# HKUST-Aerial-Robotics/VINS-Mobile

Measured on AMD Instinct MI355X. Metric: VIO frames/sec (KLT+window solve), 640x480/150 feats/W=10, higher is better.
Workload: dtype f64 (solve) / u8+i32+f32 (KLT)

## Files before the change

### vins-mobile_amd/abi.py

```python
import ctypes as C
import os

import numpy as np

VIO_OK = 0
VIO_EINVAL, VIO_ENODEV, VIO_ENOMEM, VIO_ECAP, VIO_ESTATE, VIO_ETIMEOUT = -1, -2, -3, -4, -5, -6
VIO_MAX_PRIOR_BLOCKS = 96
VIO_MAX_TRACE = 64
VIO_INIT_BA_MAX_FRAMES = 32
VIO_BLOCK_POSE, VIO_BLOCK_SPEEDBIAS, VIO_BLOCK_EXPOSE = 0, 1, 2
VIO_MARGIN_OLD, VIO_MARGIN_SECOND_NEW, VIO_MARGIN_NONE = 0, 1, 2
STAGES = ["setup_imu", "setup_prior", "eval_prior", "eval_imu", "eval_proj", "scale", "schur", "rhs", "cholesky",
          "tri_solve", "quad_form", "dogleg", "cost_eval", "new2old", "marg_build", "marg_chol", "total",
          "p_zero", "p_fact", "p_gram", "p_feat", "c_potrf", "c_trsm", "imu_raw", "c_wait", "q_w", "backsolve",
          "c_ahead", "tr_vec", "m_prior", "m_imu", "m_fact", "m_gram", "d0", "d1", "d2", "d3", "d4", "d5",
          "v_gd", "v_dot", "v_step", "v_plus", "v_gmax", "v_rest", "b_init", "b_pose", "b_asp", "b_band", "b_gn",
          "e_head", "e_copy", "e_h0dx", "e_tail", "x0", "x1", "x2", "x3"]

_dp = C.POINTER(C.c_double)
_ip = C.POINTER(C.c_int32)


class VioConfig(C.Structure):
    _fields_ = [
        ("window_size", C.c_int32), ("max_features", C.c_int32), ("max_factors", C.c_int32),
        ("max_iterations", C.c_int32), ("image_rows", C.c_int32), ("image_cols", C.c_int32),
        ("max_corners", C.c_int32), ("min_dist", C.c_int32), ("freq", C.c_int32),
        ("lk_win", C.c_int32), ("lk_levels", C.c_int32), ("lk_max_iters", C.c_int32),
        ("lk_eps", C.c_double), ("lk_min_eig", C.c_double), ("quality_level", C.c_double),
        ("f_threshold", C.c_double), ("f_confidence", C.c_double),
        ("fx", C.c_double), ("fy", C.c_double), ("cx", C.c_double), ("cy", C.c_double),
        ("gravity", C.c_double), ("acc_n", C.c_double), ("acc_w", C.c_double),
        ("gyr_n", C.c_double), ("gyr_w", C.c_double), ("cauchy_a", C.c_double),
    ]


def hip_runtime(lib=None):
    lib = lib or load_product()
    buf, n = C.create_string_buffer(4096), C.c_int32()
    lib.vio_hip_runtime(buf, 4096, C.byref(n))
    return [p for p in buf.value.decode().split(";") if p]


def host_pool_width():
    lib = load_product()
    n = C.c_int32(0)
    return int(lib.vio_host_pool_width(C.byref(n))), int(n.value)


def default_config(**kw):
    c = VioConfig(
        window_size=10, max_features=1000, max_factors=8192, max_iterations=10,
        image_rows=640, image_cols=480, max_corners=70, min_dist=30, freq=3,
        lk_win=21, lk_levels=3, lk_max_iters=30, lk_eps=0.01, lk_min_eig=1e-4,
        quality_level=0.01, f_threshold=1.0, f_confidence=0.99,
        fx=526.600, fy=526.678, cx=243.481, cy=315.280,
        gravity=9.805, acc_n=0.5, acc_w=0.002, gyr_n=0.2, gyr_w=4.0e-5, cauchy_a=1.0)
    for k, v in kw.items():
        setattr(c, k, v)
    return c


class VioPreintegration(C.Structure):
    _fields_ = [
        ("sum_dt", C.c_double), ("delta_p", C.c_double * 3), ("delta_q", C.c_double * 4),
        ("delta_v", C.c_double * 3), ("linearized_ba", C.c_double * 3),
        ("linearized_bg", C.c_double * 3), ("jacobian", C.c_double * 225),
        ("covariance", C.c_double * 225),
    ]


PREINT_DOUBLES = C.sizeof(VioPreintegration) // 8


class VioPrior(C.Structure):
    _fields_ = [
        ("n", C.c_int32), ("n_blocks", C.c_int32),
        ("block_kind", C.c_int32 * VIO_MAX_PRIOR_BLOCKS),
        ("block_index", C.c_int32 * VIO_MAX_PRIOR_BLOCKS),
        ("block_offset", C.c_int32 * VIO_MAX_PRIOR_BLOCKS),
        ("block_x0", _dp), ("linearized_jacobians", _dp), ("linearized_residuals", _dp),
    ]


class VioWindow(C.Structure):
    _fields_ = [
        ("window_size", C.c_int32), ("n_features", C.c_int32), ("n_factors", C.c_int32),
        ("marginalization_flag", C.c_int32),
        ("pose", _dp), ("speed_bias", _dp), ("ex_pose", _dp), ("inv_depth", _dp),
        ("factor_host", _ip), ("factor_target", _ip), ("factor_feature", _ip),
        ("factor_pts_i", _dp), ("factor_pts_j", _dp),
        ("preint", C.POINTER(VioPreintegration)), ("prior", C.POINTER(VioPrior)),
        ("loop_frame", C.c_int32), ("loop_pose", _dp),
        ("use_origin_override", C.c_int32), ("origin_yaw_deg", C.c_double),
        ("origin_p", C.c_double * 3),
        ("raw_pose", _dp), ("raw_speed_bias", _dp), ("raw_inv_depth", _dp),
        ("next_prior", C.POINTER(VioPrior)),
        ("resident_prior", C.c_int32),
    ]

# ... 481 lines not shown
```

### vins-mobile_amd/csrc/solver_core.h

```cpp
#pragma once

#include <math.h>
#include <stdint.h>

#include <type_traits>

#include "solve_trace.h"
#include "vio_math.h"

#include "spmd.h"
#include "factors.h"
#include "mfma_tiles.h"

namespace vio {

constexpr int kBS = 15;
constexpr int kSS = kSB * kSB;
constexpr int kAW = 18;
constexpr int kAS = kSB * kAW;

struct WinView {
  int W, P, F, M, np, nblk, has_loop, loop_frame, marg_flag, max_iter;
  int prior_n, prior_nb;
  int Fpad;
// ... 200 lines not shown
  const int need = (n + 4 * kStrip - 1) / (4 * kStrip);
  nparts = nparts < need ? need : (nparts > 8 ? 8 : nparts);
  const int per = (n + nparts - 1) / nparts;
  VIO_PARFOR(q, n * nparts) {
    const int part = q / n, c = q - part * n;
    const int k0 = part * per, k1 = k0 + per < n ? k0 + per : n;
    double xs[kStrip], s = 0;
    for (int b0 = k0; b0 < k1; b0 += kStrip) {
      const int nb = k1 - b0 < kStrip ? k1 - b0 : kStrip;
#pragma unroll
      for (int j = 0; j < kStrip; j++) xs[j] = M[(size_t)(b0 + (j < nb ? j : 0)) * n + c];
      VIO_SCHED_FENCE();
#pragma unroll
      for (int j = 0; j < kStrip; j++) s += (j < nb ? xs[j] : 0.0) * x[b0 + (j < nb ? j : 0)];
    }
    if (k1 > k0) add(c, s);
  }
}


template <class MP>
VIO_DEV void setup_imu_info_gj(const Ctx &cx, const WinView &v, MP mbox) {
  const int W = v.W;
  const int tid_ = VIO_TID(cx), j = tid_ & 31, slot = tid_ >> 5, nslots = cx.nt >> 5;
  for (int f0 = 0; f0 < W; f0 += nslots) {
    const int f = f0 + slot;
    const bool act = f < W && j < 30;
    const int fc = f < W ? f : 0;
    auto mb = mbox + slot * 32;
    double x[15];
#pragma unroll
    for (int r = 0; r < 15; r++)
      x[r] = j < 15 ? v.preint[fc * kPreintDoubles + 242 + r * 15 + (j < 15 ? j : 0)] : (double)(j - 15 == r);
#pragma unroll
    for (int c = 0; c < 15; c++) {
      if (j == c) {
        int piv = c;
        double best = fabs(x[c]);
#pragma unroll
        for (int r = c + 1; r < 15; r++)
          if (fabs(x[r]) > best) best = fabs(x[r]), piv = r;
#pragma unroll
        for (int r = 0; r < 15; r++) mb[r] = x[r];
        mb[15] = (double)piv;
      }
      __builtin_amdgcn_fence(__ATOMIC_RELEASE, "wavefront");
      __builtin_amdgcn_wave_barrier();
      __builtin_amdgcn_fence(__ATOMIC_ACQUIRE, "wavefront");
      const int piv = (int)mb[15];
      double m[15];
#pragma unroll
      for (int r = 0; r < 15; r++) m[r] = mb[r];
      __builtin_amdgcn_wave_barrier();
      double xp = x[c], mp = m[c];
#pragma unroll
      for (int r = 0; r < 15; r++) {
        if (r == piv) xp = x[r], mp = m[r];
      }
#pragma unroll
      for (int r = 0; r < 15; r++) {
        if (r == piv && r != c) x[r] = x[c], m[r] = m[c];
      }
      const double d = mp;
      x[c] = xp / d;
#pragma unroll
      for (int r = 0; r < 15; r++) {
        if (r != c) {
          const double fac = m[r];
          if (fac != 0.0) x[r] -= fac * x[c];
        }
      }
    }
    if (act && j >= 15) {
      const int cc = j - 15;
#pragma unroll
      for (int rr = 0; rr < 15; rr++)
        if (rr >= cc) v.imu_info[f * 225 + rr * 15 + cc] = x[rr], v.imu_info[f * 225 + cc * 15 + rr] = x[rr];
    }
  }
  VIO_SYNC();
}

template <class WK>
VIO_DEV void setup_prior(const Ctx &cx, const WinView &v, WK &w) {
  const int n = v.prior_n;
  if (n <= 0) return;
  VIO_PARFOR(a, n) w.prcol[a] = -1;
  VIO_SYNC();
  VIO_PARFOR(b, v.prior_nb) {
    int kind = v.pr_kind[b], idx = v.pr_index[b], o = v.pr_offset[b];
    if (kind == 0)
      for (int k = 0; k < 6; k++) w.prcol[o + k] = (idx << 8) | k;
    else if (kind == 1)
      for (int k = 0; k < 9; k++) w.prcol[o + k] = (idx << 8) | (6 + k);
  }
  const bool stage = (size_t)n * n <= (size_t)w.nstage;
  auto Js = w.stage;
  if (stage) {
    VIO_PARFOR(q, n * n) Js[q] = v.pr_J[q];
    VIO_SYNC();
  }
  {
    const int tid_ = VIO_TID(cx), wave = __builtin_amdgcn_readfirstlane(tid_ >> 6), nw = cx.nt >> 6, lane = tid_ & 63;
    const int li = lane & 15, kq = lane >> 4;
    const int nt16 = (n + 15) >> 4, ntiles = nt16 * (nt16 + 1) / 2, ksteps = (n + 3) >> 2;
    for (int t = wave; t < ntiles; t += nw) {
      int ti = 0;
      while ((ti + 1) * (ti + 2) / 2 <= t) ti++;
      const int tj = t - ti * (ti + 1) / 2;
      const int ca = 16 * ti + li, cb = 16 * tj + li;
      const bool va = ca < n, vb = cb < n;
      const int oa = va ? ca : 0, ob = vb ? cb : 0;
      v4d acc0 = {0.0, 0.0, 0.0, 0.0}, acc1 = {0.0, 0.0, 0.0, 0.0};
      constexpr int kChunk = 8;
      for (int s0 = 0; s0 < ksteps; s0 += kChunk) {
        double av[kChunk], bv[kChunk];
#pragma unroll
        for (int j = 0; j < kChunk; j++) {
          const int k = 4 * (s0 + j) + kq, kc = k < n ? k : 0;
          if (stage) av[j] = Js[kc * n + oa], bv[j] = Js[kc * n + ob];
          else av[j] = v.pr_J[kc * n + oa], bv[j] = v.pr_J[kc * n + ob];
        }
        __builtin_amdgcn_sched_barrier(0);
#pragma unroll
        for (int j = 0; j < kChunk; j++) {
          const bool vk = 4 * (s0 + j) + kq < n;
          av[j] = (va && vk) ? av[j] : 0.0, bv[j] = (vb && vk) ? bv[j] : 0.0;
        }
#pragma unroll
        for (int j = 0; j < kChunk; j += 2) acc0 = mfma_f64(av[j], bv[j], acc0), acc1 = mfma_f64(av[j + 1], bv[j + 1], acc1);
      }
      acc0 += acc1;
#pragma unroll
      for (int r = 0; r < 4; r++) {
        const int a = 16 * ti + kq + 4 * r, b = cb;
        if (a < n && b < n) {
          v.prH0[a * n + b] = acc0[r];
          if (ti != tj) v.prH0[b * n + a] = acc0[r];
        }
      }
    }
  }
  VIO_PARFOR(a, n) {
    double s = 0;
    if (stage) {
      for (int k = 0; k < n; k++) s = fma(Js[k * n + a], v.pr_r[k], s);
    } else {
      for (int k = 0; k < n; k++) s = fma(v.pr_J[k * n + a], v.pr_r[k], s);
    }
    v.prb0[a] = s;
  }
  const int napp = (int)tri_doubles(v.nrows), nband = 2 * v.P * kSS;
  VIO_PARFOR(q, kSB * v.jp) v.Apri[q] = 0.0;
  VIO_PARFOR(q, napp + nband) v.AppPr[q] = 0.0;
  VIO_SYNC();
  VIO_PARFOR(q, n * n) {
    const int a = q / n, b = q - a * n, pa = w.prcol[a], pb = w.prcol[b];
    if (pa < 0 || pb < 0 || pa < pb) continue;
    const int fr = pa >> 8, cr = pa & 255, fc = pb >> 8, cc = pb & 255;
    const double x = v.prH0[q];
    if (cr < 6 && cc < 6) v.AppPr[tri_at(6 * fr + cr, 6 * fc + cc)] = x;
    else if (cr >= 6 && cc >= 6) {
      if (fr == fc) v.AppPr[napp + fr * kSS + (cr - 6) * kSB + (cc - 6)] = x;
      else if (fr - fc == 1) v.AppPr[napp + v.P * kSS + fr * kSS + (cc - 6) * kSB + (cr - 6)] = x;
    } else if (cr >= 6) v.Apri[(cr - 6) * v.jp + 6 * fc + cc] = x;
    else v.Apri[(cc - 6) * v.jp + 6 * fr + cr] = x;
  }
  VIO_SYNC();
}

template <class MP>
VIO_DEV void setup_imu_info(const Ctx &cx, const WinView &v, MP mbox) {
  const int W = v.W;
  VIO_PARFOR(q, W * 450) v.imu_J[q] = 0.0;
  constexpr int kLd = 17, kTile = 16 * kLd + 16;
  const int tid_ = VIO_TID(cx), wave = __builtin_amdgcn_readfirstlane(tid_ >> 6), nw = cx.nt >> 6, lane = tid_ & 63;
  const int n = lane & 15, kq = lane >> 4;
  auto T = mbox + wave * kTile;
  auto ldv = T + 16 * kLd;
  bool all_good = true;
  if (cx.tid == 0) mbox[nw * kTile] = 0.0;
  VIO_SYNC();
  for (int f = wave; f < W; f += nw) {
    const double *cov = v.preint + f * kPreintDoubles + 242;
    double c4[4];
#pragma unroll
    for (int r = 0; r < 4; r++) {
      const int row = kq + 4 * r, hi = row > n ? row : n, lo = row > n ? n : row;
      c4[r] = cov[(hi < 15 ? hi : 0) * 15 + (lo < 15 ? lo : 0)];
    }
#pragma unroll
    for (int r = 0; r < 4; r++) {
      const int row = kq + 4 * r;
      T[row * kLd + n] = (row < 15 && n < 15) ? c4[r] : (row == n ? 1.0 : 0.0);
    }
    __builtin_amdgcn_fence(__ATOMIC_RELEASE, "wavefront");
    __builtin_amdgcn_wave_barrier();
    __builtin_amdgcn_fence(__ATOMIC_ACQUIRE, "wavefront");
    const bool good = potrf16_wave(T, T, kLd, 15, 15, false, ldv, lane);
    all_good = all_good && good;
    __builtin_amdgcn_fence(__ATOMIC_RELEASE, "wavefront");
    __builtin_amdgcn_wave_barrier();
    __builtin_amdgcn_fence(__ATOMIC_ACQUIRE, "wavefront");
    double x[4];
    const double dg = ldv[n < 15 ? n : 0];
#pragma unroll
    for (int s4 = 0; s4 < 4; s4++) x[s4] = T[(n < 15 ? n : 0) * kLd + (4 * s4 + kq)];
    VIO_SCHED_FENCE();
    v4d acc = {0.0, 0.0, 0.0, 0.0};
#pragma unroll
    for (int s4 = 0; s4 < 4; s4++) {
      const int k = 4 * s4 + kq;
      const double xv = (n < 15 && k < 15) ? (k > n ? x[s4] : (k == n ? dg : 0.0)) : 0.0;
      acc = mfma_f64(xv, xv, acc);
    }
#pragma unroll
    for (int r = 0; r < 4; r++) {
      const int row = kq + 4 * r;
      if (row < 15 && n < 15) v.imu_info[f * 225 + row * 15 + n] = acc[r];
    }
    __builtin_amdgcn_wave_barrier();
  }
  if (__builtin_amdgcn_ballot_w64(!all_good) != 0 && lane == 0) mbox[nw * kTile] = 1.0;
  VIO_SYNC();
  const bool fallback = mbox[nw * kTile] == 1.0;
  VIO_SYNC();
  if (fallback) setup_imu_info_gj(cx, v, mbox);
}

constexpr int kPanelTiles = 5;
constexpr int kGRow = 10;
constexpr int kGSlot = 2 * kGRow + 1;
constexpr int kGramPiece = 30;
constexpr int kGramMinChunk = 32;

template <class WK>
VIO_DEV int gram_chunk_slots(const Ctx &cx, const WK &w) {
  int CH = (w.nstage / kGSlot) & ~1;
  if (CH >= (int)cx.nt) CH -= CH % (int)cx.nt;
  return CH;
}

template <class WK>
VIO_DEV void build_gram_pieces(const Ctx &cx, const WinView &v, WK &w) {
  const int CH = gram_chunk_slots(cx, w), nchunks = (v.nslots + CH - 1) / CH;
  ldsi cnt = reinterpret_cast<ldsi>(w.stage);
  ldsi cc = cnt + v.npairs;
  VIO_PARFOR(c, nchunks + 1) cc[c] = 0;
  VIO_SYNC();
  VIO_PARFOR(b, v.npairs) {
    const int s0 = v.pair_s0[b], s1 = v.pair_s1[b];
    int n = 0;
    for (int c = s0 / CH; c * CH < s1; c++) {
      const int lo = s0 > c * CH ? s0 : c * CH, hi = s1 < (c + 1) * CH ? s1 : (c + 1) * CH;
      const int np_ = (hi - lo + kGramPiece - 1) / kGramPiece;
      n += np_;
#ifdef VIO_HOST_BUILD
      cc[c + 1] += np_;
#else
      __hip_atomic_fetch_add(cc + c + 1, np_, __ATOMIC_RELAXED, __HIP_MEMORY_SCOPE_WORKGROUP);
#endif
    }
    cnt[b] = n;
  }
  VIO_SYNC();
// ... 1984 lines not shown
      relin = true;
      continue;
    }
    invalid_run = 0;
    stamp(cx, ST_DOGLEG);
    const bool speculate = last_ok;
    const int npose7 = (v.P + v.has_loop) * 7, o_sb = 7 * (v.P + 1), o_f = o_sb + 9 * v.P, o_v = o_f + F, nv = v.nblk * kBS;
    double step_norm, cand_norm;
    {
      double d2 = 0, c2 = 0, dummy3 = 0;
      plus_in_place(cx, fresh(), w, w.t2, w.tf, v.stash, o_sb, o_f, d2, c2);
      VIO_PARFOR(q, F)
        v.stash[o_v + 3 * nv + q] = w.gf[q], v.stash[o_v + 3 * nv + F + q] = w.hff[q], v.stash[o_v + 3 * nv + 2 * F + q] = w.gnf[q];
      VIO_PARFOR(i, np) v.stash[o_v + i] = w.gp[i], v.stash[o_v + nv + i] = w.dp[i], v.stash[o_v + 2 * nv + i] = w.gnp[i];
      block_sum3(cx, d2, c2, dummy3);
      step_norm = sqrt(d2), cand_norm = sqrt(c2);
      stamp(cx, ST_V_PLUS);
    }
    double cand_cost = evaluate(cx, fresh(), w, w.xpose, w.xsb, w.xfeat, speculate, true, false, !speculate);
    if (!isfinite(cand_cost)) cand_cost = 1.7976931348623157e308;
    auto restore_iterate = [&]() {
      VIO_PARFOR(q, npose7) w.xpose[q] = v.stash[q];
      VIO_PARFOR(q, v.P * 9) w.xsb[q] = v.stash[o_sb + q];
      VIO_PARFOR(q, F) w.xfeat[q] = v.stash[o_f + q];
    };
    if (step_norm <= 1e-8 * (x_norm + 1e-8)) {
      restore_iterate();
      termination = 1;
      break;
    }
    double cost_change = x_cost - cand_cost;
    if (fabs(cost_change) <= 1e-6 * x_cost) {
      restore_iterate();
      termination = 1;
      break;
    }
    const double rho = step_quality(ev, cand_cost, model_cost_change);
    if (rho > 1e-3) {
      x_norm = cand_norm;
      x_cost = cand_cost;
      if (rho < 0.25) radius *= 0.5;
      if (rho > 0.75) radius = fmax(radius, 3.0 * dogleg_step_norm);
      mu = fmax(min_mu, 2.0 * mu / mu_inc);
      reuse = false;
      ev.current_cost = cand_cost, ev.accumulated_candidate_model_cost_change += model_cost_change, ev.accumulated_reference_model_cost_change += model_cost_change;
      if (ev.current_cost < ev.minimum_cost) ev.minimum_cost = ev.current_cost, ev.candidate_cost = ev.current_cost, ev.accumulated_candidate_model_cost_change = 0;
      else if (ev.current_cost > ev.candidate_cost) ev.candidate_cost = ev.current_cost, ev.accumulated_candidate_model_cost_change = 0;
      ev.reference_cost = ev.candidate_cost, ev.accumulated_reference_model_cost_change = ev.accumulated_candidate_model_cost_change;
      last_ok = true;
      n_ok++;
      recorded = it + 1, min_rec = fmin(min_rec, x_cost);
      if (speculate) {
        gmax = grad_max_norm();
        if (cx.tid == 0) trace.record(it, x_cost, radius, step_norm, rho, gmax, true, true);
        stamp(cx, ST_V_GMAX);
      } else {
        relin = true, relin_reuse = true, rec_pending = true;
        rec_it = it, rec_step_norm = step_norm, rec_rho = rho;
      }
    } else {
      radius *= 0.5;
      reuse = true;
      last_ok = false;
      n_bad++;
      if (cx.tid == 0) trace.record(it, cand_cost, radius, step_norm, rho, 0.0, true, false);
      recorded = it + 1, min_rec = fmin(min_rec, cand_cost);
      restore_iterate();
      if (speculate) {
        VIO_PARFOR(q, F) w.gf[q] = v.stash[o_v + 3 * nv + q], w.hff[q] = v.stash[o_v + 3 * nv + F + q], w.gnf[q] = v.stash[o_v + 3 * nv + 2 * F + q];
        VIO_PARFOR(i, np) w.gp[i] = v.stash[o_v + i], w.dp[i] = v.stash[o_v + nv + i], w.gnp[i] = v.stash[o_v + 2 * nv + i];
      }
      VIO_SYNC();
      stamp(cx, ST_V_REST);
    }
  }
  if (cx.tid == 0) trace.finish(recorded, termination, n_ok, n_bad, min_rec);
  VIO_SYNC();
}

template <class WK>
VIO_DEV void init_band_reach(const Ctx &cx, const WinView &v, WK &w) {
  VIO_PARFOR(k, v.P) {
    int lo = 6 * (k > 0 ? k - 1 : 0), pr = 0;
    for (int b = 0; b < v.prior_nb; b++)
      if (v.pr_kind[b] == 1 && v.pr_index[b] == k) lo = 0, pr = 1;
    w.sbr[2 * k] = lo, w.sbr[2 * k + 1] = pr;
  }
}

#ifndef VIO_HOST_BUILD
template <class WK>
VIO_DEV void coop_helper(const Ctx &cx, const WinView &v, WK &w) {
  const CoopLayout L = CoopLayout::make(v.Pcap, v.Fcap, v.nblk_cap);
  const int np = v.np, F = v.F, nFr = v.P + v.has_loop;
  const size_t fs = ((size_t)v.Fcap + 7) & ~(size_t)7;
  double *part = v.coop + L.o_part + (size_t)(cx.member - 1) * L.part;
  init_band_reach(cx, v, w);
  VIO_SYNC();
  for (;;) {
    const int cmd = coop_wait_cmd(cx, v);
    if (cmd == COOP_EVAL) {
      VIO_PARFOR(q, 7 * nFr) w.xpose[q] = v.coop[L.o_pose + q];
      VIO_PARFOR(q, F) w.xfeat[q] = v.coop[L.o_feat + q];
      VIO_PARFOR(q, 7) w.ex[q] = v.coop[L.o_ex + q];
      VIO_PARFOR(q, np) w.gp[q] = 0.0;
      VIO_PARFOR(q, F) {
        w.gf[q] = 0.0, w.hff[q] = 0.0;
        w.cfeat[q] = w.stf[q] = w.gnf[q] = w.tf[q] = w.ef[q] = w.einv[q] = 0.0;
      }
      VIO_PARFOR(q, nFr * 36) w.ppd[q] = 0.0;
      VIO_SYNC();
      VIO_PARFOR(i, nFr + 1) {
        const bool is_ex = i == nFr;
        double R[9];
        if (is_ex) qtoR(Quat{w.ex[3], w.ex[4], w.ex[5], w.ex[6]}, R);
        else qtoR(Quat{w.xpose[7 * i + 3], w.xpose[7 * i + 4], w.xpose[7 * i + 5], w.xpose[7 * i + 6]}, R);
        auto dst = w.rot + 9 * (is_ex ? v.P + 1 : i);
        for (int k = 0; k < 9; k++) dst[k] = R[k];
      }
      VIO_SYNC();
      const double cost = block_sum(cx, projections_jac(cx, v, w, w.xpose, w.xfeat, true, cx.member, cx.coop, false));
      ldsd whv[6] = {w.cfeat, w.stf, w.gnf, w.tf, w.ef, w.einv};
      VIO_PARFOR(q, np) part[L.p_gp + q] = w.gp[q];
      VIO_PARFOR(q, nFr * 36) part[L.p_ppd + q] = w.ppd[q];
      VIO_PARFOR(f, F) {
        part[L.p_f + f] = w.hff[f], part[L.p_f + fs + f] = w.gf[f];
#pragma unroll
        for (int c = 0; c < 6; c++) part[L.p_f + (2 + c) * fs + f] = whv[c][f];
      }
      if (cx.tid == 0) part[L.p_cost] = cost;
    } else if (cmd == COOP_SCHUR) {
      VIO_PARFOR(f, F) w.einv[f] = v.coop[L.o_einv + f], w.tf[f] = v.coop[L.o_tf + f];
      VIO_SYNC();
      schur_general(cx, v, w, cx.member, cx.coop);
    } else if (cmd == COOP_SYRK) {
      band_syrk_share(cx, v, w, cx.member, cx.coop);
    } else {
      break;
    }
    coop_done(cx, v);
  }
}
#endif

template <bool REGS, int NW, class WK, class VP, class WP>
VIO_DEV void solve_window(const Ctx &cx, const WinView &v, WK &w, const VP &fresh, const WP &fresh_work) {
  const int P = v.P, F = v.F;
  VIO_PARFOR(q, P * 7) w.xpose[q] = v.pose0[q];
  VIO_PARFOR(q, P * 9) w.xsb[q] = v.sb0[q];
  VIO_PARFOR(q, F) w.xfeat[q] = v.feat0[q];
  VIO_PARFOR(q, 7) w.ex[q] = v.ex[q];
  if (v.has_loop) VIO_PARFOR(q, 7) w.xpose[7 * P + q] = v.pose0[7 * v.loop_frame + q];
  VIO_PARFOR(q, v.nblk * kBS) w.t1[q] = 0.0, w.t2[q] = 0.0;
  if (cx.tid == 0) w.flag[0] = w.flag[1] = w.flag[2] = w.flag[3] = 0;
  init_band_reach(cx, v, w);
  VIO_SYNC();
  if (cx.prof && cx.tid == cx.prof_tid) {
    for (int q = 0; q < ST_COUNT; q++) cx.lprof[q] = 0;
    cx.lprof[ST_COUNT - 1] = clock64();
    cx.lprof[ST_TOTAL] = -cx.lprof[ST_COUNT - 1];
  }
  VIO_PARFOR(q, v.nslots) v.sfact[q] = -1;
  VIO_SYNC();
  VIO_PARFOR(q, v.nslots) v.srec_i[q] = -1;
  VIO_SYNC();
  VIO_PARFOR(k, v.M) {
    const int sl = v.fslot[k];
    v.sfact[sl] = k;
    v.srec_i[sl] = v.fhost[k] | (v.ftarget[k] << 8) | (v.ffeat[k] << 16);
    double *d = v.srec_d + 6 * (size_t)sl;
    for (int c = 0; c < 3; c++) d[c] = v.pts_i[3 * k + c], d[3 + c] = v.pts_j[3 * k + c];
  }
  build_gram_pieces(cx, v, w);
  VIO_PARFOR(f, F) w.fh[f] = v.fstart[f + 1] > v.fstart[f] ? v.fhost[v.fstart[f]] : -1;
  VIO_PARFOR(q, (int)tri_doubles(v.nrows)) v.PP[q] = 0.0;
  setup_imu_info(cx, fresh(), w.stage);
  stamp(cx, ST_SETUP_IMU);
  setup_prior(cx, fresh(), w);
  stamp(cx, ST_SETUP_PRIOR);

  minimize<REGS, NW>(cx, v, w, fresh, fresh_work);

  VIO_PARFOR(q, P * 7) v.raw_pose[q] = w.xpose[q];
  VIO_PARFOR(q, P * 9) v.raw_sb[q] = w.xsb[q];
  VIO_PARFOR(q, F) v.raw_feat[q] = w.xfeat[q];
  if (v.has_loop) VIO_PARFOR(q, 7) v.out_loop[q] = w.xpose[7 * P + q];
  VIO_SYNC();
  double R0in[9], ypr0[3], R00[9], ypr00[3], rot_diff[9];
  qtoR(qnormalized(qfrom_pose(v.pose0)), R0in);
  R2ypr(R0in, ypr0);
  double origin_yaw = v.use_origin ? v.origin_yaw : ypr0[0];
  double op[3] = {v.use_origin ? v.origin_p[0] : v.pose0[0], v.use_origin ? v.origin_p[1] : v.pose0[1],
                  v.use_origin ? v.origin_p[2] : v.pose0[2]};
  qtoR(qfrom_pose(w.xpose), R00);
  R2ypr(R00, ypr00);
  double yd[3] = {origin_yaw - ypr00[0], 0, 0};
  ypr2R(yd, rot_diff);
  double p0[3] = {w.xpose[0], w.xpose[1], w.xpose[2]};
  VIO_SYNC();
  VIO_PARFOR(i, P) {
    auto pp = w.xpose + 7 * i, sbv = w.xsb + 9 * i;
    double Rq[9], Rs[9], d[3] = {pp[0] - p0[0], pp[1] - p0[1], pp[2] - p0[2]}, Ps[3], Vs[3];
    qtoR(qnormalized(qfrom_pose(pp)), Rq);
    mat3mul(rot_diff, Rq, Rs);
    mat3vec(rot_diff, d, Ps);
    double vv[3] = {sbv[0], sbv[1], sbv[2]};
    mat3vec(rot_diff, vv, Vs);
    Quat q = RtoQ(Rs);
    auto po = w.cpose + 7 * i, so = w.csb + 9 * i;
    for (int k = 0; k < 3; k++) po[k] = Ps[k] + op[k], so[k] = Vs[k];
    po[3] = q.x, po[4] = q.y, po[5] = q.z, po[6] = q.w;
    for (int k = 3; k < 9; k++) so[k] = sbv[k];
  }
  VIO_PARFOR(f, F) {
    double estimated_depth = 1.0 / w.xfeat[f];
    w.cfeat[f] = 1. / estimated_depth;
  }
  VIO_SYNC();
  VIO_PARFOR(q, P * 7) v.out_pose[q] = w.cpose[q], w.xpose[q] = w.cpose[q];
  VIO_PARFOR(q, P * 9) v.out_sb[q] = w.csb[q], w.xsb[q] = w.csb[q];
  VIO_PARFOR(q, F) v.out_feat[q] = w.cfeat[q], w.xfeat[q] = w.cfeat[q];
  VIO_SYNC();
  stamp(cx, ST_NEW2OLD);
}


}
```

### vins-mobile_amd/csrc/spmd.h

```cpp
#pragma once

#include <math.h>
#include <stdint.h>

#include "vio_math.h"

#if defined(VIO_EMUL) || defined(VIO_SIMT)
#define VIO_HOST_BUILD 1
#endif
#ifdef VIO_HOST_BUILD
#define VIO_DEV inline
#define VIO_ATOMIC_ADD(p, v) ::vio::atomic_add((p), (v))
#else
#define VIO_DEV __device__ __forceinline__
#define VIO_ATOMIC_ADD(p, v) ::vio::atomic_add((p), (v))
#endif
#if defined(VIO_EMUL)
#define VIO_SYNC() ((void)0)
#define VIO_SYNC_LDS() ((void)0)
#elif defined(VIO_SIMT)
#define VIO_SYNC() __syncthreads()
#define VIO_SYNC_LDS() __syncthreads()
#else
#define VIO_SYNC() __syncthreads()
#define VIO_SYNC_LDS()                                                      \
  do {                                                                      \
    __builtin_amdgcn_fence(__ATOMIC_RELEASE, "workgroup", "local");         \
    __builtin_amdgcn_s_barrier();                                           \
    __builtin_amdgcn_fence(__ATOMIC_ACQUIRE, "workgroup", "local");         \
  } while (0)
#endif
#ifdef VIO_HOST_BUILD
#define VIO_TID(cx) ((int)(cx).tid)
#else
#define VIO_TID(cx) ::vio::hw_tid((cx).wave64)
#endif
#define VIO_PARFOR(i, n) for (int i = VIO_TID(cx); i < (int)(n); i += (int)cx.nt)
#ifdef VIO_HOST_BUILD
#define VIO_OPAQUE(x) (x)
#else
#define VIO_OPAQUE(x) ::vio::opaque_tid(x)
#endif

#ifdef VIO_HOST_BUILD
#define VIO_AS3
#else
#define VIO_AS3 __attribute__((address_space(3)))
#endif

namespace vio {

#ifndef VIO_HOST_BUILD
__device__ __forceinline__ int opaque_tid(int t) {
  asm volatile("" : "+v"(t));
  return t;
}
__device__ __forceinline__ int hw_tid(int wave64) {
  int t;
  asm volatile("v_mbcnt_lo_u32_b32 %0, -1, %1\n\tv_mbcnt_hi_u32_b32 %0, -1, %0" : "=v"(t) : "s"(wave64));
  return t;
}
#endif

typedef VIO_AS3 double *ldsd;
typedef const VIO_AS3 double *cldsd;
typedef VIO_AS3 int *ldsi;

#ifdef VIO_HOST_BUILD
inline void atomic_add(double *p, double v) { *p += v; }
inline void atomic_add_noret(double *p, double v) { *p += v; }
#else
__device__ __forceinline__ void atomic_add_noret(double *p, double v) {
  (void)__hip_atomic_fetch_add(p, v, __ATOMIC_RELAXED, __HIP_MEMORY_SCOPE_AGENT);
}
__device__ __forceinline__ void atomic_add(ldsd p, double v) {
  __hip_atomic_fetch_add(p, v, __ATOMIC_RELAXED, __HIP_MEMORY_SCOPE_WORKGROUP);
}
__device__ __forceinline__ void atomic_add(double *p, double v) {
  __hip_atomic_fetch_add(p, v, __ATOMIC_RELAXED, __HIP_MEMORY_SCOPE_WORKGROUP);
}
#endif

enum Stage {
  ST_SETUP_IMU = 0, ST_SETUP_PRIOR, ST_EVAL_PRIOR, ST_EVAL_IMU, ST_EVAL_PROJ, ST_SCALE, ST_SCHUR, ST_RHS, ST_CHOL,
  ST_TRISOLVE, ST_QUADFORM, ST_DOGLEG, ST_COST_EVAL, ST_NEW2OLD, ST_MARG_BUILD, ST_MARG_CHOL, ST_TOTAL,
  ST_P_ZERO, ST_P_FACT, ST_P_GRAM, ST_P_FEAT,
  ST_C_POTRF, ST_C_TRSM,
  ST_IMU_RAW,
  ST_C_WAIT, ST_Q_W, ST_BACKSOLVE, ST_C_AHEAD,
  ST_TR_VEC,
  ST_M_PRIOR, ST_M_IMU, ST_M_FACT, ST_M_GRAM,
  ST_D0, ST_D1, ST_D2, ST_D3, ST_D4, ST_D5,
  ST_V_GD,
  ST_V_DOT, ST_V_STEP,
  ST_V_PLUS,
  ST_V_GMAX,
  ST_V_REST,
  ST_B_INIT, ST_B_POSE, ST_B_ASP, ST_B_BAND, ST_B_GN,
  ST_E_HEAD, ST_E_COPY, ST_E_H0DX, ST_E_TAIL,
  ST_X0, ST_X1, ST_X2, ST_X3,
  ST_COUNT = 64
};

struct Ctx {
  int tid, nt;
  int wave64 = 0;
  ldsd red;
  mutable int red_phase = 0;
  long long *prof;
  int wrot = 0;
  int prof_tid = 0;
  VIO_AS3 long long *lprof;
  int coop = 1, member = 0;
  unsigned coop_spin = 1u << 24;
  mutable unsigned coop_seq = 0;
};

VIO_DEV void stamp(const Ctx &cx, int stage) {
#if !defined(VIO_EMUL)
  if (cx.prof && cx.tid == cx.prof_tid) {
    long long t = clock64();
    cx.lprof[stage] += t - cx.lprof[ST_COUNT - 1];
    cx.lprof[ST_COUNT - 1] = t;
  }
#else
  (void)cx, (void)stage;
#endif
}

#ifndef VIO_EMUL
template <int CTRL, int ROWMASK>
__device__ __forceinline__ double dpp_move_f64(double v) {
  int lo = __builtin_amdgcn_update_dpp(0, __double2loint(v), CTRL, ROWMASK, 0xf, false);
  int hi = __builtin_amdgcn_update_dpp(0, __double2hiint(v), CTRL, ROWMASK, 0xf, false);
  return __hiloint2double(hi, lo);
}
__device__ __forceinline__ double wave_sum_f64(double v) {
  v += dpp_move_f64<0x111, 0xf>(v);
  v += dpp_move_f64<0x112, 0xf>(v);
  v += dpp_move_f64<0x114, 0xf>(v);
  v += dpp_move_f64<0x118, 0xf>(v);
  v += dpp_move_f64<0x142, 0xa>(v);
  v += dpp_move_f64<0x143, 0xc>(v);
  return __hiloint2double(__builtin_amdgcn_readlane(__double2hiint(v), 63), __builtin_amdgcn_readlane(__double2loint(v), 63));
}
__device__ __forceinline__ double wave_max_f64(double v) {
  v = fmax(v, dpp_move_f64<0x111, 0xf>(v));
  v = fmax(v, dpp_move_f64<0x112, 0xf>(v));
  v = fmax(v, dpp_move_f64<0x114, 0xf>(v));
  v = fmax(v, dpp_move_f64<0x118, 0xf>(v));
  v = fmax(v, dpp_move_f64<0x142, 0xa>(v));
  v = fmax(v, dpp_move_f64<0x143, 0xc>(v));
  return __hiloint2double(__builtin_amdgcn_readlane(__double2hiint(v), 63), __builtin_amdgcn_readlane(__double2loint(v), 63));
}
#endif
VIO_DEV double block_sum(const Ctx &cx, double v) {
#ifdef VIO_EMUL
  return v;
#else
  const int nw = cx.nt >> 6;
  ldsd red = cx.red + (cx.red_phase ^= 1) * 3 * nw;
  v = wave_sum_f64(v);
  if ((cx.tid & 63) == 0) red[cx.tid >> 6] = v;
  VIO_SYNC();
  double s = 0;
  for (int w = 0; w < nw; w++) s += red[w];
  return s;
#endif
}
VIO_DEV void block_sum3(const Ctx &cx, double &a, double &b, double &c) {
#ifndef VIO_EMUL
  const int nw = cx.nt >> 6;
  ldsd red = cx.red + (cx.red_phase ^= 1) * 3 * nw;
  a = wave_sum_f64(a), b = wave_sum_f64(b), c = wave_sum_f64(c);
  if ((cx.tid & 63) == 0) red[cx.tid >> 6] = a, red[nw + (cx.tid >> 6)] = b, red[2 * nw + (cx.tid >> 6)] = c;
  VIO_SYNC();
  a = b = c = 0;
  for (int w = 0; w < nw; w++) a += red[w], b += red[nw + w], c += red[2 * nw + w];
#else
  (void)cx, (void)a, (void)b, (void)c;
#endif
}
VIO_DEV double block_max(const Ctx &cx, double v) {
// ... 34 lines not shown
```

Baseline: 198,300.

## Fuse prior scatter into Gram tile epilogue and batch window setup loads

In the REGS path, the prior Hessian placement into AppPr/Apri now happens directly in the MFMA tile write-out, which removes a separate n*n scatter pass and one barrier. The staging copy, the slot-record initialization and the state copies are restructured so several loads are issued before their stores, and the column map is built earlier. Several barriers between the initialization loops are merged. The change also adds profiling stamps, and zeroing and scattering now share one barrier region, which relies on disjoint addresses.

```diff
diff --git a/vins-mobile_amd/abi.py b/vins-mobile_amd/abi.py
--- a/vins-mobile_amd/abi.py
+++ b/vins-mobile_amd/abi.py
@@ -15,7 +15,7 @@
           "p_zero", "p_fact", "p_gram", "p_feat", "c_potrf", "c_trsm", "imu_raw", "c_wait", "q_w", "backsolve",
           "c_ahead", "tr_vec", "m_prior", "m_imu", "m_fact", "m_gram", "d0", "d1", "d2", "d3", "d4", "d5",
           "v_gd", "v_dot", "v_step", "v_plus", "v_gmax", "v_rest", "b_init", "b_pose", "b_asp", "b_band", "b_gn",
-          "e_head", "e_copy", "e_h0dx", "e_tail", "x0", "x1", "x2", "x3"]
+          "e_head", "e_copy", "e_h0dx", "e_tail", "x0", "x1", "x2", "x3", "s0", "s1", "s2", "s3"]
 
 _dp = C.POINTER(C.c_double)
 _ip = C.POINTER(C.c_int32)
diff --git a/vins-mobile_amd/csrc/solver_core.h b/vins-mobile_amd/csrc/solver_core.h
--- a/vins-mobile_amd/csrc/solver_core.h
+++ b/vins-mobile_amd/csrc/solver_core.h
@@ -306,11 +306,7 @@
 }
 
 template <class WK>
-VIO_DEV void setup_prior(const Ctx &cx, const WinView &v, WK &w) {
-  const int n = v.prior_n;
-  if (n <= 0) return;
-  VIO_PARFOR(a, n) w.prcol[a] = -1;
-  VIO_SYNC();
+VIO_DEV void prior_column_map(const Ctx &cx, const WinView &v, WK &w) {
   VIO_PARFOR(b, v.prior_nb) {
     int kind = v.pr_kind[b], idx = v.pr_index[b], o = v.pr_offset[b];
     if (kind == 0)
@@ -318,12 +314,57 @@
     else if (kind == 1)
       for (int k = 0; k < 9; k++) w.prcol[o + k] = (idx << 8) | (6 + k);
   }
+}
+
+VIO_DEV void prior_place(const WinView &v, int napp, int pa, int pb, double x) {
+  const int fr = pa >> 8, cr = pa & 255, fc = pb >> 8, cc = pb & 255;
+  if (cr < 6 && cc < 6) v.AppPr[tri_at(6 * fr + cr, 6 * fc + cc)] = x;
+  else if (cr >= 6 && cc >= 6) {
+    if (fr == fc) v.AppPr[napp + fr * kSS + (cr - 6) * kSB + (cc - 6)] = x;
+    else if (fr - fc == 1) v.AppPr[napp + v.P * kSS + fr * kSS + (cc - 6) * kSB + (cr - 6)] = x;
+  } else if (cr >= 6) v.Apri[(cr - 6) * v.jp + 6 * fc + cc] = x;
+  else v.Apri[(cc - 6) * v.jp + 6 * fr + cr] = x;
+}
+
+template <bool ACC, class WK>
+VIO_DEV void setup_prior(const Ctx &cx, const WinView &v, WK &w) {
+  const int n = v.prior_n;
+  if (n <= 0) return;
+  const int napp = (int)tri_doubles(v.nrows), nband = 2 * v.P * kSS;
   const bool stage = (size_t)n * n <= (size_t)w.nstage;
   auto Js = w.stage;
-  if (stage) {
-    VIO_PARFOR(q, n * n) Js[q] = v.pr_J[q];
+  if constexpr (ACC) {
+    VIO_PARFOR(q, kSB * v.jp) v.Apri[q] = 0.0;
+    VIO_PARFOR(q, napp + nband) v.AppPr[q] = 0.0;
+    constexpr int kU = 12;
+    const int tid_ = VIO_TID(cx), nt_ = (int)cx.nt, nn = n * n;
+    if (stage) {
+      for (int q0 = tid_; q0 < nn; q0 += kU * nt_) {
+        double x[kU];
+#pragma unroll
+        for (int u = 0; u < kU; u++) {
+          const int q = q0 + u * nt_;
+          x[u] = v.pr_J[q < nn ? q : 0];
+        }
+        VIO_SCHED_FENCE();
+#pragma unroll
+        for (int u = 0; u < kU; u++) {
+          const int q = q0 + u * nt_;
+          if (q < nn) Js[q] = x[u];
+        }
+      }
+    }
     VIO_SYNC();
-  }
+  } else {
+    VIO_PARFOR(a, n) w.prcol[a] = -1;
+    VIO_SYNC();
+    prior_column_map(cx, v, w);
+    if (stage) {
+      VIO_PARFOR(q, n * n) Js[q] = v.pr_J[q];
+      VIO_SYNC();
+    }
+  }
+  stamp(cx, ST_D5);
   {
     const int tid_ = VIO_TID(cx), wave = __builtin_amdgcn_readfirstlane(tid_ >> 6), nw = cx.nt >> 6, lane = tid_ & 63;
     const int li = lane & 15, kq = lane >> 4;
@@ -351,20 +392,36 @@
           const bool vk = 4 * (s0 + j) + kq < n;
           av[j] = (va && vk) ? av[j] : 0.0, bv[j] = (vb && vk) ? bv[j] : 0.0;
         }
-#pragma unroll
-        for (int j = 0; j < kChunk; j += 2) acc0 = mfma_f64(av[j], bv[j], acc0), acc1 = mfma_f64(av[j + 1], bv[j + 1], acc1);
+        if constexpr (ACC) {
+#pragma unroll
+          for (int j = 0; j < kChunk; j += 2) {
+            if (s0 + j < ksteps) acc0 = mfma_f64(av[j], bv[j], acc0);
+            if (s0 + j + 1 < ksteps) acc1 = mfma_f64(av[j + 1], bv[j + 1], acc1);
+          }
+        } else {
+#pragma unroll
+          for (int j = 0; j < kChunk; j += 2) acc0 = mfma_f64(av[j], bv[j], acc0), acc1 = mfma_f64(av[j + 1], bv[j + 1], acc1);
+        }
       }
       acc0 += acc1;
+      const int pb0 = (ACC && vb) ? w.prcol[cb] : -1;
 #pragma unroll
       for (int r = 0; r < 4; r++) {
         const int a = 16 * ti + kq + 4 * r, b = cb;
         if (a < n && b < n) {
-          v.prH0[a * n + b] = acc0[r];
-          if (ti != tj) v.prH0[b * n + a] = acc0[r];
-        }
-      }
-    }
-  }
+          const double x = acc0[r];
+          v.prH0[a * n + b] = x;
+          if (ti != tj) v.prH0[b * n + a] = x;
+          if constexpr (ACC) {
+            int pa = w.prcol[a], pb = pb0;
+            if (ti != tj && pa < pb) pa = pb0, pb = w.prcol[a];
+            if (pb >= 0 && pa >= pb) prior_place(v, napp, pa, pb, x);
+          }
+        }
+      }
+    }
+  }
+  stamp(cx, ST_S0);
   VIO_PARFOR(a, n) {
     double s = 0;
     if (stage) {
@@ -374,21 +431,17 @@
     }
     v.prb0[a] = s;
   }
-  const int napp = (int)tri_doubles(v.nrows), nband = 2 * v.P * kSS;
-  VIO_PARFOR(q, kSB * v.jp) v.Apri[q] = 0.0;
-  VIO_PARFOR(q, napp + nband) v.AppPr[q] = 0.0;
-  VIO_SYNC();
-  VIO_PARFOR(q, n * n) {
-    const int a = q / n, b = q - a * n, pa = w.prcol[a], pb = w.prcol[b];
-    if (pa < 0 || pb < 0 || pa < pb) continue;
-    const int fr = pa >> 8, cr = pa & 255, fc = pb >> 8, cc = pb & 255;
-    const double x = v.prH0[q];
-    if (cr < 6 && cc < 6) v.AppPr[tri_at(6 * fr + cr, 6 * fc + cc)] = x;
-    else if (cr >= 6 && cc >= 6) {
-      if (fr == fc) v.AppPr[napp + fr * kSS + (cr - 6) * kSB + (cc - 6)] = x;
-      else if (fr - fc == 1) v.AppPr[napp + v.P * kSS + fr * kSS + (cc - 6) * kSB + (cr - 6)] = x;
-    } else if (cr >= 6) v.Apri[(cr - 6) * v.jp + 6 * fc + cc] = x;
-    else v.Apri[(cc - 6) * v.jp + 6 * fr + cr] = x;
+  stamp(cx, ST_S1);
+  if constexpr (!ACC) {
+    VIO_PARFOR(q, kSB * v.jp) v.Apri[q] = 0.0;
+    VIO_PARFOR(q, napp + nband) v.AppPr[q] = 0.0;
+    VIO_SYNC();
+    stamp(cx, ST_S2);
+    VIO_PARFOR(q, n * n) {
+      const int a = q / n, b = q - a * n, pa = w.prcol[a], pb = w.prcol[b];
+      if (pa < 0 || pb < 0 || pa < pb) continue;
+      prior_place(v, napp, pa, pb, v.prH0[q]);
+    }
   }
   VIO_SYNC();
 }
@@ -405,6 +458,7 @@
   bool all_good = true;
   if (cx.tid == 0) mbox[nw * kTile] = 0.0;
   VIO_SYNC();
+  stamp(cx, ST_S3);
   for (int f = wave; f < W; f += nw) {
     const double *cov = v.preint + f * kPreintDoubles + 242;
     double c4[4];
@@ -2555,8 +2609,19 @@
 VIO_DEV void init_band_reach(const Ctx &cx, const WinView &v, WK &w) {
   VIO_PARFOR(k, v.P) {
     int lo = 6 * (k > 0 ? k - 1 : 0), pr = 0;
-    for (int b = 0; b < v.prior_nb; b++)
-      if (v.pr_kind[b] == 1 && v.pr_index[b] == k) lo = 0, pr = 1;
+    constexpr int kB = 8;
+    for (int b0 = 0; b0 < v.prior_nb; b0 += kB) {
+      int kind[kB], idx[kB];
+#pragma unroll
+      for (int j = 0; j < kB; j++) {
+        const int b = b0 + j < v.prior_nb ? b0 + j : b0;
+        kind[j] = v.pr_kind[b], idx[j] = v.pr_index[b];
+      }
+      VIO_SCHED_FENCE();
+#pragma unroll
+      for (int j = 0; j < kB; j++)
+        if (kind[j] == 1 && idx[j] == k) lo = 0, pr = 1;
+    }
     w.sbr[2 * k] = lo, w.sbr[2 * k + 1] = pr;
   }
 }
@@ -2619,37 +2684,90 @@
 template <bool REGS, int NW, class WK, class VP, class WP>
 VIO_DEV void solve_window(const Ctx &cx, const WinView &v, WK &w, const VP &fresh, const WP &fresh_work) {
   const int P = v.P, F = v.F;
-  VIO_PARFOR(q, P * 7) w.xpose[q] = v.pose0[q];
-  VIO_PARFOR(q, P * 9) w.xsb[q] = v.sb0[q];
-  VIO_PARFOR(q, F) w.xfeat[q] = v.feat0[q];
-  VIO_PARFOR(q, 7) w.ex[q] = v.ex[q];
-  if (v.has_loop) VIO_PARFOR(q, 7) w.xpose[7 * P + q] = v.pose0[7 * v.loop_frame + q];
-  VIO_PARFOR(q, v.nblk * kBS) w.t1[q] = 0.0, w.t2[q] = 0.0;
-  if (cx.tid == 0) w.flag[0] = w.flag[1] = w.flag[2] = w.flag[3] = 0;
-  init_band_reach(cx, v, w);
-  VIO_SYNC();
   if (cx.prof && cx.tid == cx.prof_tid) {
     for (int q = 0; q < ST_COUNT; q++) cx.lprof[q] = 0;
     cx.lprof[ST_COUNT - 1] = clock64();
     cx.lprof[ST_TOTAL] = -cx.lprof[ST_COUNT - 1];
   }
-  VIO_PARFOR(q, v.nslots) v.sfact[q] = -1;
-  VIO_SYNC();
-  VIO_PARFOR(q, v.nslots) v.srec_i[q] = -1;
-  VIO_SYNC();
-  VIO_PARFOR(k, v.M) {
-    const int sl = v.fslot[k];
-    v.sfact[sl] = k;
-    v.srec_i[sl] = v.fhost[k] | (v.ftarget[k] << 8) | (v.ffeat[k] << 16);
-    double *d = v.srec_d + 6 * (size_t)sl;
-    for (int c = 0; c < 3; c++) d[c] = v.pts_i[3 * k + c], d[3 + c] = v.pts_j[3 * k + c];
-  }
+  if constexpr (REGS) {
+    const int t = VIO_TID(cx), nt_ = (int)cx.nt;
+    const double xp = v.pose0[t < P * 7 ? t : 0], xs = v.sb0[t < P * 9 ? t : 0], xe = v.ex[t < 7 ? t : 0];
+    const double xf = *(t < F ? v.feat0 + t : v.pose0);
+    const double xl = v.pose0[(v.has_loop ? 7 * v.loop_frame : 0) + (t < 7 ? t : 0)];
+    VIO_SCHED_FENCE();
+    if (t < P * 7) w.xpose[t] = xp;
+    if (t < P * 9) w.xsb[t] = xs;
+    if (t < F) w.xfeat[t] = xf;
+    if (t < 7) w.ex[t] = xe;
+    if (v.has_loop && t < 7) w.xpose[7 * P + t] = xl;
+    for (int q = t + nt_; q < P * 7; q += nt_) w.xpose[q] = v.pose0[q];
+    for (int q = t + nt_; q < P * 9; q += nt_) w.xsb[q] = v.sb0[q];
+    for (int q = t + nt_; q < F; q += nt_) w.xfeat[q] = v.feat0[q];
+  } else {
+    VIO_PARFOR(q, P * 7) w.xpose[q] = v.pose0[q];
+    VIO_PARFOR(q, P * 9) w.xsb[q] = v.sb0[q];
+    VIO_PARFOR(q, F) w.xfeat[q] = v.feat0[q];
+    VIO_PARFOR(q, 7) w.ex[q] = v.ex[q];
+    if (v.has_loop) VIO_PARFOR(q, 7) w.xpose[7 * P + q] = v.pose0[7 * v.loop_frame + q];
+  }
+  VIO_PARFOR(q, v.nblk * kBS) w.t1[q] = 0.0, w.t2[q] = 0.0;
+  if (cx.tid == 0) w.flag[0] = w.flag[1] = w.flag[2] = w.flag[3] = 0;
+  init_band_reach(cx, v, w);
+  if constexpr (REGS) {
+    VIO_PARFOR(a, v.prior_n) w.prcol[a] = -1;
+    VIO_PARFOR(q, v.nslots) v.sfact[q] = -1, v.srec_i[q] = -1;
+    VIO_SYNC();
+    stamp(cx, ST_X1);
+    prior_column_map(cx, v, w);
+    constexpr int kT = 4;
+    const int t = VIO_TID(cx), nt_ = (int)cx.nt, M = v.M;
+    for (int k0 = t; k0 < M; k0 += kT * nt_) {
+      int sl[kT], rec[kT];
+      double pt[kT][6];
+#pragma unroll
+      for (int u = 0; u < kT; u++) {
+        const int k = k0 + u * nt_, kc = k < M ? k : 0;
+        sl[u] = v.fslot[kc];
+        rec[u] = v.fhost[kc] | (v.ftarget[kc] << 8) | (v.ffeat[kc] << 16);
+#pragma unroll
+        for (int c = 0; c < 3; c++) pt[u][c] = v.pts_i[3 * kc + c], pt[u][3 + c] = v.pts_j[3 * kc + c];
+      }
+      VIO_SCHED_FENCE();
+#pragma unroll
+      for (int u = 0; u < kT; u++) {
+        const int k = k0 + u * nt_;
+        if (k < M) {
+          v.sfact[sl[u]] = k;
+          v.srec_i[sl[u]] = rec[u];
+          double *d = v.srec_d + 6 * (size_t)sl[u];
+#pragma unroll
+          for (int c = 0; c < 6; c++) d[c] = pt[u][c];
+        }
+      }
+    }
+  } else {
+    VIO_SYNC();
+    stamp(cx, ST_X1);
+    VIO_PARFOR(q, v.nslots) v.sfact[q] = -1;
+    VIO_SYNC();
+    VIO_PARFOR(q, v.nslots) v.srec_i[q] = -1;
+    VIO_SYNC();
+    VIO_PARFOR(k, v.M) {
+      const int sl = v.fslot[k];
+      v.sfact[sl] = k;
+      v.srec_i[sl] = v.fhost[k] | (v.ftarget[k] << 8) | (v.ffeat[k] << 16);
+      double *d = v.srec_d + 6 * (size_t)sl;
+      for (int c = 0; c < 3; c++) d[c] = v.pts_i[3 * k + c], d[3 + c] = v.pts_j[3 * k + c];
+    }
+  }
+  stamp(cx, ST_X2);
   build_gram_pieces(cx, v, w);
+  stamp(cx, ST_X3);
   VIO_PARFOR(f, F) w.fh[f] = v.fstart[f + 1] > v.fstart[f] ? v.fhost[v.fstart[f]] : -1;
   VIO_PARFOR(q, (int)tri_doubles(v.nrows)) v.PP[q] = 0.0;
   setup_imu_info(cx, fresh(), w.stage);
   stamp(cx, ST_SETUP_IMU);
-  setup_prior(cx, fresh(), w);
+  setup_prior<REGS>(cx, fresh(), w);
   stamp(cx, ST_SETUP_PRIOR);
 
   minimize<REGS, NW>(cx, v, w, fresh, fresh_work);
diff --git a/vins-mobile_amd/csrc/spmd.h b/vins-mobile_amd/csrc/spmd.h
--- a/vins-mobile_amd/csrc/spmd.h
+++ b/vins-mobile_amd/csrc/spmd.h
@@ -99,6 +99,7 @@
   ST_B_INIT, ST_B_POSE, ST_B_ASP, ST_B_BAND, ST_B_GN,
   ST_E_HEAD, ST_E_COPY, ST_E_H0DX, ST_E_TAIL,
   ST_X0, ST_X1, ST_X2, ST_X3,
+  ST_S0, ST_S1, ST_S2, ST_S3,
   ST_COUNT = 64
 };
 
```

After: 200,600 (median of 6 runs). 1.01x the previous value.
